# mir-group/allegro

Hardware: NVIDIA H100
Metric: atom-steps/sec (energy+forces) (higher is better)
Workload: dtype f32

## Files before the change

allegro_b200/_lib.py:

```python
from __future__ import annotations

import ctypes as C
import os
from typing import Optional, Sequence, Tuple

import torch

from . import build as _build

AB2_F64, AB2_F32, AB2_BF16 = 0, 1, 2
ACT_NONE, ACT_SILU, ACT_MUL_DSILU = 0, 1, 2
EPI_NONE, EPI_MUL_DSILU = 0, 1
NL_SILU, NL_MISH, NL_GELU = 1, 2, 3
NOT_ELIGIBLE = -1
MAX_SEG = 4

DTYPE_ENUM = {torch.float64: AB2_F64, torch.float32: AB2_F32, torch.bfloat16: AB2_BF16}
ACC_DTYPE = {torch.float64: torch.float64, torch.float32: torch.float32, torch.bfloat16: torch.float32}

_LIB: Optional[C.CDLL] = None

_vp, _i64, _i32, _dbl = C.c_void_p, C.c_int64, C.c_int, C.c_double

_SIGNATURES = {
# ... 2 lines not shown
    "ab2_last_error": ([], C.c_char_p),
    "ab2_set_option": ([C.c_char_p, _i32], C.c_int),
    "ab2_op_scatter_env": ([_i32, _i64, _i64, _dbl, _vp, _vp, _vp, _vp], C.c_int),
    "ab2_op_contract": ([_i32, _i32, _i64, _i32, _i32, _i32, _i32, _i32, _vp, _vp, _vp, _vp, _vp, _vp, _vp], C.c_int),
    "ab2_op_gather_rows": ([_i32, _i64, _i64, _dbl, _vp, _vp, _vp, _vp], C.c_int),
    "ab2_op_contract_wgrad": ([_i32, _i64, _i32, _i32, _i32, _i32, _i32, _vp, _vp, _vp, _vp, _vp, _vp, _vp], C.c_int),
    "ab2_sh_fwd": ([_i32, _i32, _i64, _vp, _vp, _vp], C.c_int),
    "ab2_sh_bwd": ([_i32, _i32, _i64, _vp, _vp, _vp, _i32, _vp], C.c_int),
    "ab2_linear": ([_i32, _i64, _i32, _i32, _i32, _vp, _vp, _vp, _vp, _vp, _i32, _vp, _vp, _i32, _vp, _vp, _vp, _vp, _i32, _vp, _i64, _vp], C.c_int),
    "ab2_linear_nl": ([_i32, _i64, _i32, _i32, _i32, _vp, _vp, _vp, _vp, _vp, _i32, _vp, _vp, _i32, _vp, _vp, _vp, _vp, _i32, _vp, _i64, _vp, _i32], C.c_int),
    "ab2_linear_packed_bytes": ([_i32, _i32, _i32], C.c_int64),
    "ab2_linear_pack": ([_i32, _i32, _i32, _vp, _vp, _vp], C.c_int),
    "ab2_mlp2_readout": ([_i32, _i32, _i64, _i32, _i32, _i32, _i32, _vp, _i64, _vp, _i64, _vp, _i64, _vp, _i64, _vp, _i64, _vp, _i64, _vp, _vp, _vp], C.c_int),
    "ab2_mlp2": ([_i32, _i32, _i64, _i32, _i32, _i32, _i32, _vp, _vp, _vp, _vp, _vp, _vp, _vp, _i64, _i32, _vp, _vp, _vp, _vp, _vp], C.c_int),
    "ab2_mlp2_nl": ([_i32, _i32, _i64, _i32, _i32, _i32, _i32, _vp, _vp, _vp, _vp, _vp, _vp, _vp, _i64, _i32, _vp, _vp, _vp, _vp, _vp, _i32], C.c_int),
    "ab2_mlp2_readout_nl": ([_i32, _i32, _i64, _i32, _i32, _i32, _i32, _vp, _i64, _vp, _i64, _vp, _i64, _vp, _i64, _vp, _i64, _vp, _i64, _vp, _vp, _vp, _i32],
                            C.c_int),
    "ab2_env_sum": ([_i32, _i32, _i64, _i32, _vp, _vp, _vp, _i64, _dbl, _vp, _vp], C.c_int),
    "ab2_env_bwd": ([_i32, _i32, _i64, _i64, _i32, _vp, _vp, _vp, _vp, _i64, _vp, _dbl, _vp, _i64, _vp, _vp], C.c_int),
    "ab2_tp_fwd": ([_i32, _i32, _i64, _i64, _i32, _i32, _i32, _i32, _vp, _vp, _vp, _vp, _vp, _vp, _i32, _vp, _vp, _i64, _vp, _vp], C.c_int),
    "ab2_tp_bwd": ([_i32, _i32, _i64, _i64, _i32, _i32, _i32, _i32, _vp, _vp, _vp, _vp, _vp, _vp, _i32, _vp, _vp, _i64, _vp, _vp, _vp, _i64, _vp, _vp, _vp], C.c_int),
    "ab2_tp_chain_fwd": ([_i32, _i32, _i64, _i64, _i32, _vp, _vp, _vp, _vp, _vp, _vp, _vp, _vp, _vp, _vp], C.c_int),
    "ab2_tp_chain_bwd": ([_i32, _i32, _i64, _i64, _i32, _vp, _vp, _vp, _vp, _vp, _vp, _vp, _vp, _vp, _vp, _vp, _vp, _vp, _vp], C.c_int),
    "ab2_edge_sum": ([_i32, _i64, _vp, _vp, _dbl, _vp, _vp], C.c_int),
    "ab2_edge_sum_bwd": ([_i32, _i64, _vp, _vp, _dbl, _vp, _vp], C.c_int),
    "ab2_force_scatter": ([_i32, _i64, _i64, _i64, _vp, _vp, _vp, _vp, _vp, _vp], C.c_int),
    "ab2_force_virial_scatter": ([_i32, _i64, _i64, _i64, _vp, _vp, _vp, _vp, _vp, _vp, _vp, _vp], C.c_int),
    "ab2_transpose_ui": ([_i32, _i64, _i32, _i32, _vp, _vp, _i32, _vp], C.c_int),
    "ab2_edge_vec": ([_i32, _i32, _i64, _vp, _vp, _vp, _vp, _vp, _vp], C.c_int),
    "ab2_radial_fwd": ([_i32, _i64, _i32, _i32, _dbl, _vp, _vp, _vp, _vp, _vp, _i32, _vp, _vp, _vp, _vp, _vp, _vp], C.c_int),
    "ab2_radial_pq_fwd": ([_i32, _i64, _i32, _i32, _dbl, _vp, _vp, _vp, _vp, _vp, _i32, _vp, _vp, _vp, _vp], C.c_int),
    "ab2_radial_pq_bwd": ([_i32, _i64, _i32, _i32, _dbl, _vp, _vp, _vp, _vp, _vp, _i32, _vp, _vp, _vp, _vp, _vp, _vp], C.c_int),
    "ab2_radial_pq_bwd_nl": ([_i32, _i64, _i32, _i32, _dbl, _vp, _vp, _vp, _vp, _vp, _i32, _vp, _vp, _vp, _vp, _vp, _vp, _i32], C.c_int),
    "ab2_zbl": ([_i32, _i64, _i32, _dbl, _dbl, _vp, _vp, _vp, _vp, _vp, _vp, _vp, _vp, _vp], C.c_int),
    "ab2_p2p_mailbox_bytes": ([_i32, _i32], C.c_int64),
    "ab2_p2p_alloc": ([_i64, C.POINTER(C.c_void_p)], C.c_int),
    "ab2_p2p_free": ([_vp], C.c_int),
    "ab2_p2p_get_handle": ([_vp, _vp], C.c_int),
    "ab2_p2p_open_handle": ([_vp, C.POINTER(C.c_void_p)], C.c_int),
    "ab2_p2p_close_handle": ([_vp], C.c_int),
    "ab2_p2p_error": ([_vp, _i32, _i32, _vp], C.c_int),
    "ab2_p2p_begin": ([_vp, _vp], C.c_int),
    "ab2_p2p_push_rows": ([_i32, _i32, _i32, _vp, _vp, _i32, _dbl, _vp, _i32, _i32, _vp, _vp, _vp], C.c_int),
    "ab2_p2p_push_rows_v": ([_i32, _i32, _i32, _vp, _vp, _i32, _dbl, _dbl, _dbl, _vp, _i32, _i32, _vp, _vp, _vp], C.c_int),
    "ab2_p2p_wait_unpack": ([_i32, _i32, _i32, _vp, _i32, _i32, _vp, _i32, _vp, _vp, _i32, _vp], C.c_int),
    "ab2_p2p_allreduce_energy": ([_vp, _i32, _i32, _i32, _vp, _vp, _vp, _vp, _vp], C.c_int),
    "ab2_p2p_mailbox_bytes_ex": ([_i32, _i32, _i32], C.c_int64),
    "ab2_p2p_push_rows_w": ([_i32, _i32, _vp, _vp, _i32, _vp, _i32, _i32, _vp, _vp, _vp], C.c_int),
    "ab2_p2p_wait_unpack_w": ([_i32, _i32, _vp, _i32, _i32, _vp, _i32, _vp, _vp, _vp, _vp], C.c_int),
    "ab2_p2p_allreduce_vec": ([_vp, _i32, _i32, _i32, _i32, _vp, _vp, _vp, _vp, _vp], C.c_int),
    "ab2_slab_plan_count": ([_i32, _i32, _i64, _vp, _vp, _vp, _i32, _i32, _dbl, _dbl, _dbl, _vp, _vp, _vp], C.c_int),
    "ab2_slab_plan_fill": ([_i64, _vp, _vp, _vp, _vp, _vp, _vp], C.c_int),
    "ab2_slab_plan_count_lattice": ([_i32, _i32, _i64, _vp, _vp, _vp, _i32, _i32, _dbl, _dbl, _vp, _vp, _vp], C.c_int),
    "ab2_nl_bin": ([_i32, _i64, _vp, _vp, _vp, _vp, _vp, _dbl, _vp, _vp], C.c_int),
    "ab2_nl_count": ([_i32, _i64, _vp, _vp, _vp, _vp, _vp, _dbl, _vp, _vp, _vp, _vp], C.c_int),
    "ab2_nl_fill": ([_i32, _i64, _vp, _vp, _vp, _vp, _vp, _dbl, _vp, _vp, _vp, _vp, _vp, _vp], C.c_int),
    "ab2_nl_lattice_bin": ([_i32, _i64, _vp, _vp, _vp, _vp, _vp, _vp, _dbl, _vp, _vp], C.c_int),
    "ab2_nl_lattice_count": ([_i32, _i64, _vp, _vp, _vp, _vp, _vp, _vp, _dbl, _vp, _vp, _vp, _vp], C.c_int),
    "ab2_nl_lattice_fill": ([_i32, _i64, _vp, _vp, _vp, _vp, _vp, _vp, _dbl, _vp, _vp, _vp, _vp, _vp, _vp], C.c_int),
    "ab2_radial_bwd": ([_i32, _i64, _i32, _i32, _dbl, _vp, _vp, _vp, _vp, _vp, _i32, _vp, _vp, _vp, _vp, _vp, _vp, _vp], C.c_int),
    "ab2_nl_frames_count": ([_i32, _i64, _i64, _vp, _vp, _vp, _vp, _vp, _vp, _dbl, _vp, _vp], C.c_int),
    "ab2_nl_frames_fill": ([_i32, _i64, _i64, _vp, _vp, _vp, _vp, _vp, _vp, _dbl, _vp, _vp, _vp, _vp], C.c_int),
    "ab2_nl_prune_count": ([_i32, _i64, _i64, _i32, _vp, _vp, _vp, _vp, _vp, _vp, _vp, _vp], C.c_int),
    "ab2_nl_prune_fill": ([_i32, _i64, _i64, _i32, _vp, _vp, _vp, _vp, _vp, _vp, _vp, _vp, _vp, _vp], C.c_int),
    "ab2_frame_scratch_elems": ([_i64, _i64], C.c_int64),
    "ab2_frame_sum": ([_i32, _i64, _i64, _vp, _vp, _vp, _i64, _vp, _vp], C.c_int),
# ... 686 lines not shown
    n_centres = n if n_centres is None else int(n_centres)
    dt = DTYPE_ENUM[pos.dtype]
    pos = _contig(pos, "pos")
    cell_id = torch.empty(n, dtype=torch.int32, device=pos.device)
    with _timed(name + "_bin"):
        _check(bin_fn(dt, n, _ptr(pos), *geom, _ptr(cell_id), _stream()))
    order = torch.argsort(cell_id, stable=True).to(torch.int32)
    ncells = ncell[0] * ncell[1] * ncell[2]
    cell_start = torch.zeros(ncells + 1, dtype=torch.int32, device=pos.device)
    cell_start[1:] = torch.cumsum(torch.bincount(cell_id.long(), minlength=ncells), 0).to(torch.int32)
    counts = torch.empty(n_centres, dtype=torch.int32, device=pos.device)
    with _timed(name + "_count"):
        _check(count_fn(dt, n_centres, _ptr(pos), *geom, _ptr(cell_start), _ptr(order), _ptr(counts), _stream()))
    row_ptr = torch.zeros(n_centres + 1, dtype=torch.int32, device=pos.device)
    row_ptr[1:] = torch.cumsum(counts, 0).to(torch.int32)
    E = int(row_ptr[-1])
    nbr = torch.empty(E, dtype=torch.int32, device=pos.device)
    shift = torch.empty(E, 3, dtype=pos.dtype, device=pos.device)
    if E:
        with _timed(name + "_fill"):
            _check(fill_fn(dt, n_centres, _ptr(pos), *geom, _ptr(cell_start), _ptr(order), _ptr(row_ptr), _ptr(nbr), _ptr(shift), _stream()))
    return row_ptr, nbr, shift


def radial_pq_fwd(dtype, S: int, p_cut: float, vec, ctr, nbr, types, rmax_table, bessel_w, PQ) -> torch.Tensor:
    E = ctr.shape[0]
    out = torch.empty(E, S, dtype=dtype, device=vec.device)
    with _timed("radial_fwd"):
        _check(load().ab2_radial_pq_fwd(DTYPE_ENUM[dtype], E, S, bessel_w.numel(), float(p_cut), _ptr(vec), _ptr(ctr), _ptr(nbr), _ptr(types),
                                        _ptr(rmax_table), rmax_table.shape[0], _ptr(bessel_w), _ptr(_contig(PQ, "PQ")), _ptr(out), _stream()))
    return out


def radial_pq_bwd(dtype, S: int, p_cut: float, vec, ctr, nbr, types, rmax_table, bessel_w, PQ, g_out, aux, gvec, nonlin: int = NL_SILU):
    E = ctr.shape[0]
    args = (DTYPE_ENUM[dtype], E, S, bessel_w.numel(), float(p_cut), _ptr(vec), _ptr(ctr), _ptr(nbr), _ptr(types), _ptr(rmax_table),
            rmax_table.shape[0], _ptr(bessel_w), _ptr(_contig(PQ, "PQ")), _ptr(_contig(g_out, "g_out")),
            _ptr(_contig(aux, "aux")) if aux is not None else None, _ptr(gvec), _stream())
    with _timed("radial_bwd"):
        _check(load().ab2_radial_pq_bwd(*args) if nonlin == NL_SILU else load().ab2_radial_pq_bwd_nl(*args, nonlin))


def _slab_plan(mode: int, pos: torch.Tensor, image: Optional[torch.Tensor], box, rank: int, world: int, width: float, jump: float,
               r_list: float, n_lists: int, rows=None):
    n = pos.shape[0]
    if rows is not None:
        rowsa = (C.c_double * 9)(*[float(v) for row in rows for v in row])
        count = lambda cls, counts: load().ab2_slab_plan_count_lattice(
            DTYPE_ENUM[pos.dtype], mode, n, _ptr(_contig(pos, "pos")) if n else None, _ptr(image) if n else None, rowsa, int(rank), int(world),
            float(jump), float(r_list), _ptr(cls), _ptr(counts), _stream())
        if n == 0:
            _check(count(None, None))
    else:
        boxa = (C.c_double * 3)(*[float(b) for b in box])
        count = lambda cls, counts: load().ab2_slab_plan_count(
            DTYPE_ENUM[pos.dtype], mode, n, _ptr(_contig(pos, "pos")), _ptr(image), boxa, int(rank), int(world), float(width), float(jump),
            float(r_list), _ptr(cls), _ptr(counts), _stream())
    if n == 0:
        return [torch.empty(0, dtype=torch.int64, device=pos.device) for _ in range(n_lists)], 0
    nblk = (n + 255) // 256
    cls = torch.empty(n, dtype=torch.uint8, device=pos.device)
    counts = torch.empty(nblk, 4, dtype=torch.int32, device=pos.device)
    with _timed("slab_plan_count"):
        _check(count(cls, counts))
    incl = torch.cumsum(counts, 0, dtype=torch.int32)
    offsets = (incl - counts).contiguous()
    lists = [torch.empty(n, dtype=torch.int64, device=pos.device) for _ in range(n_lists)]
    ptrs = [_ptr(t) for t in lists] + [None] * (3 - n_lists)
    with _timed("slab_plan_fill"):
        _check(load().ab2_slab_plan_fill(n, _ptr(cls), _ptr(offsets), *ptrs, _stream()))
    totals = incl[-1].tolist()
    return [t[:c] for t, c in zip(lists, totals)], int(totals[3])

# ... 343 lines not shown
```

allegro_b200/csrc/linear_tc.cu:

```cuda
#include <cuda.h>

#include <type_traits>

#include "common.cuh"

extern int g_ab2_opt_linear_tc;
extern int g_ab2_opt_linear_tma;
extern int g_ab2_opt_tc_debug;

namespace {

constexpr int BM = 128;
constexpr int KC = 32;
constexpr int NSTAGE = 4;
constexpr int RAW_STAGE = 256 * 4 * 16;
constexpr int EPI_LD = 40;
constexpr int NCONS = 8;
constexpr int EPI_BYTES = NCONS * 16 * EPI_LD * 4;
constexpr int STAGE_HALF = BM * KC * 2;
constexpr int NPROD = 8;
constexpr int NTHREADS = (NPROD + NCONS) * 32;
constexpr int MAX_W_BYTES = 128 * 1024;
constexpr int MAX_K = 512;
constexpr int MAX_N = 128;
constexpr int MAX_CHUNK = MAX_N / 32;
constexpr int TAIL_BARS = 2 * NSTAGE * 8, TAIL_CHUNK = MAX_CHUNK * 32, TAIL_KMAP = (MAX_K / 8) * 16;
constexpr int TAIL_BYTES = TAIL_BARS + TAIL_CHUNK + 2 * TAIL_KMAP;

struct TcSeg {
    const void* ptr;
    int64_t ld;
    int width;
    int accum;
    const void* aux;
    int64_t aux_ld;
};

// ... 815 lines not shown
    const int w_bytes = 2 * w_half;
    const int stage_bytes = 2 * STAGE_HALF;
    const int raw_slot = TMA_BOX_BYTES * (p.has_aux ? 2 : 1);
    uint8_t* sRaw = smem + ((1024u - (smem_u32(smem) & 1023u)) & 1023u);
    uint8_t* sW = sRaw + (size_t)NR * raw_slot;
    uint8_t* sA = sW + ((w_bytes + 127) & ~127);
    float* sEpi = reinterpret_cast<float*>(sA + p.nstage * stage_bytes);
    uint64_t* bars = reinterpret_cast<uint64_t*>(reinterpret_cast<uint8_t*>(sEpi) + EPI_BYTES);
    ChunkInfo* sChunk = reinterpret_cast<ChunkInfo*>(reinterpret_cast<uint8_t*>(bars) + TAIL_BARS);
    int4* sKseg = reinterpret_cast<int4*>(reinterpret_cast<uint8_t*>(sChunk) + TAIL_CHUNK);
    uint64_t* rbars = reinterpret_cast<uint64_t*>(reinterpret_cast<uint8_t*>(sKseg) + (MAX_K / 32) * 16);
    const uint32_t bar0 = smem_u32(bars), rbar0 = smem_u32(rbars);
    const int nkb = p.K / KC;

    if (threadIdx.x == 0) tma_init_bars(bar0, rbar0, WPG);
    if (threadIdx.x < MAX_K / 32) {
        sKseg[threadIdx.x] = tma_kseg_entry(p, threadIdx.x);
    } else if (threadIdx.x >= 64 && threadIdx.x < 64 + MAX_CHUNK) {
        sChunk[threadIdx.x - 64] = tc_chunk_info<TSrc>(p, (threadIdx.x - 64) * 32);
    }
    stage_w(sW, p.Wpacked, p.Wlo, w_half);
    fence_proxy_async();
    __syncthreads();
    TcCtx ctx;
    ctx.sW = sW; ctx.sA = sA; ctx.sEpi = sEpi; ctx.sChunk = sChunk; ctx.bar0 = bar0;
    ctx.nkb = nkb; ctx.stage_bytes = stage_bytes; ctx.w_half = w_half;
    const int64_t my_tiles = (p.num_tiles > blockIdx.x) ? (p.num_tiles - blockIdx.x + gridDim.x - 1) / gridDim.x : 0;
    const int64_t total = my_tiles * nkb;

    if (warp >= NPROD) {
        tc_consumer_role<TSrc, SPLIT, NCH, NL>(p, ctx, warp - NPROD, lane);
    } else {
        tma_converter_role<G, NL>(p, maps, NR, ctx, sRaw, sKseg, rbar0, total, warp, lane);
    }
}

constexpr int MLP2_MAX_H = 64;
constexpr int MLP2_CHUNK = 64;
constexpr int MLP2_MAX_CHUNKS = 4;
constexpr int MLP2_TAIL = TAIL_BARS + (1 + MLP2_MAX_CHUNKS) * TAIL_CHUNK + (MAX_K / 32) * 16 + 8 * 8;

struct Mlp2Params {
    TcParams s1;
    TcParams s2[MLP2_MAX_CHUNKS];
    int n0[MLP2_MAX_CHUNKS];
    int n2;
    int w2_npad;
    int backward;
    const float* pre;
    int64_t pre_ld;
    const float* gout1;
    int64_t gout1_ld;
    const float* w1row;
};

template <int NCH>
__device__ __forceinline__ void mlp2_stage2(const TcParams& p2, const ChunkInfo* chunks, float* stg, uint32_t h_u, uint32_t h_half, int H, uint32_t w_u,
                                            uint32_t w_half, int64_t tile, int wg, int w4, int lane) {
    float acc[16 * NCH];
    tc_mma_resident<NCH>(acc, h_u, h_half, H, w_u, w_half);
    tc_epilogue<float, NCH, false>(p2, chunks, stg, acc, tile, wg, w4, lane);
}

template <int NCH1, int NL>
__global__ void __launch_bounds__(NTHREADS, 1) mlp2_kernel(const __grid_constant__ Mlp2Params q, const __grid_constant__ TmaMaps maps, int NR) {
    constexpr int G = 2, WPG = NPROD / G;
// ... 741 lines not shown
        }
    }
    q.s2[0].Wpacked = W2_packed;
    q.s2[0].Wlo = reinterpret_cast<const uint8_t*>(W2_packed) + (size_t)w2_npad * H * 2;

    const unsigned grid = (unsigned)((num_tiles < num_sms) ? num_tiles : num_sms);
    cudaStream_t st = (cudaStream_t)stream;
    auto go = [&](auto kern) -> int {
        if (cudaFuncSetAttribute(kern, cudaFuncAttributeMaxDynamicSharedMemorySize, (int)smem) != cudaSuccess) {
            cudaGetLastError();
            return AB2_NOT_ELIGIBLE;
        }
        kern<<<grid, NTHREADS, smem, st>>>(q, maps, NR);
        AB2_CUDA_LAUNCH_CHECK();
        return 0;
    };
    return tc_with_nl(nonlin, [&](auto nl) -> int {
        constexpr int NL = decltype(nl)::value;
        switch (H / 32) {
            case 1: return go(mlp2_kernel<1, NL>);
            case 2: return go(mlp2_kernel<2, NL>);
        }
        return AB2_NOT_ELIGIBLE;
    });
}

extern "C" int ab2_mlp2(int dtype, int backward, int64_t M, int K, int H, int N, int n_a, const void* const* a_ptr, const int64_t* a_ld,
                        const int32_t* a_width, const void* W1_packed, const void* W2_packed, const void* w1_row, void* pre, int64_t pre_ld, int n_o,
                        void* const* o_ptr, const int64_t* o_ld, const int32_t* o_width, const int32_t* o_accum, void* stream) {
    return ab2_mlp2_nl(dtype, backward, M, K, H, N, n_a, a_ptr, a_ld, a_width, W1_packed, W2_packed, w1_row, pre, pre_ld, n_o, o_ptr, o_ld, o_width,
                       o_accum, stream, AB2_NL_SILU);
}

extern "C" int ab2_mlp2_readout_nl(int dtype, int backward, int64_t M, int P, int S, int U, int H, void* x, int64_t x_ld, void* s, int64_t s_ld,
                                   void* xl, int64_t xl_ld, void* pre_l, int64_t pre_l_ld, void* pre_r, int64_t pre_r_ld, void* ez, int64_t ez_ld,
                                   const void* const* w_packed, const void* w2_ro, void* stream, int nonlin) {
    AB2_CHECK_ARG(nonlin == AB2_NL_SILU || nonlin == AB2_NL_MISH || nonlin == AB2_NL_GELU, "nonlinearity");
    AB2_CHECK_ARG(P > 0 && S > 0 && U > 0 && H > 0 && M >= 0, "shape");
    AB2_CHECK_ARG(x && s && pre_l && pre_r && ez && w2_ro && w_packed && (backward || xl), "null pointer");
    AB2_CHECK_ARG(x_ld >= P && s_ld >= U && (backward || xl_ld >= S) && pre_l_ld >= H && pre_r_ld >= H && ez_ld >= 1, "leading dimension");
    if (M == 0) return 0;
    const int n_w = backward ? 3 : 4;
    auto al16 = [](const void* ptr, int64_t ld) { return (reinterpret_cast<uintptr_t>(ptr) % 16) == 0 && (ld * 4) % 16 == 0; };
    if (dtype != AB2_F32 || !g_ab2_opt_linear_tc || !g_ab2_opt_linear_tma || (!backward && !tc_encode_fn())) return AB2_NOT_ELIGIBLE;
    if (H != RO_H || S != RO_H || P % KC != 0 || U % KC != 0 || P + U > MAX_K || M >= ((int64_t)1 << 31)) return AB2_NOT_ELIGIBLE;
    if (!al16(x, x_ld) || !al16(s, s_ld) || (!backward && !al16(xl, xl_ld)) || !al16(pre_l, pre_l_ld) || !al16(pre_r, pre_r_ld) ||
        reinterpret_cast<uintptr_t>(w2_ro) % 16 != 0)
        return AB2_NOT_ELIGIBLE;
    for (int i = 0; i < n_w; ++i)
        if (!w_packed[i]) return AB2_NOT_ELIGIBLE;

    Mlp2RoParams q;
    memset(&q, 0, sizeof(q));
    const int64_t num_tiles = (M + BM - 1) / BM;
    q.P = P;
    q.w2ro = reinterpret_cast<const float*>(w2_ro);
    q.ez = reinterpret_cast<float*>(ez);
    q.ez_ld = ez_ld;
    for (int i = 0; i < n_w; ++i) q.w[i] = w_packed[i];
    TcParams& p = q.s1;
    p.M = M; p.num_tiles = num_tiles;
    auto out1 = [&](TcParams& o, void* ptr, int64_t ld, int n) {
        o.M = M; o.K = H; o.N = n; o.Npad = n; o.epi = AB2_EPI_NONE; o.num_tiles = num_tiles;
        o.n_o = 1; o.o[0].ptr = ptr; o.o[0].ld = ld; o.o[0].width = n;
    };
    int num_sms = 0, max_smem = 0;
// ... 68 lines not shown
```

allegro_b200/csrc/radial.cu:

```cuda
#include "common.cuh"

#define AB2_MAX_BESSEL 16

template <typename T>
__device__ __forceinline__ T ab2_sin(T x);
template <>
__device__ __forceinline__ float ab2_sin<float>(float x) { return sinf(x); }
template <>
__device__ __forceinline__ double ab2_sin<double>(double x) { return sin(x); }
template <typename T>
__device__ __forceinline__ T ab2_cos(T x);
template <>
__device__ __forceinline__ float ab2_cos<float>(float x) { return cosf(x); }
template <>
__device__ __forceinline__ double ab2_cos<double>(double x) { return cos(x); }
__device__ __forceinline__ float ab2_pow(float x, float p) { return powf(x, p); }
__device__ __forceinline__ double ab2_pow(double x, double p) { return pow(x, p); }

template <typename TPos, typename TAcc>
__global__ void __launch_bounds__(256) edge_vec_kernel(int64_t E, const TPos* __restrict__ pos, const int32_t* __restrict__ ctr,
                                                       const int32_t* __restrict__ nbr, const TPos* __restrict__ shift,
                                                       TAcc* __restrict__ vec) {
    const int64_t z = (int64_t)blockIdx.x * 256 + threadIdx.x;
    if (z >= E) return;
    const int64_t i = ctr[z], j = nbr[z];
#pragma unroll
    for (int a = 0; a < 3; ++a) {
        TPos d = pos[j * 3 + a] - pos[i * 3 + a];
        if (shift) d += shift[z * 3 + a];
        vec[z * 3 + a] = (TAcc)d;
    }
}

template <typename TAcc, bool GRAD>
__device__ __forceinline__ void bessel_basis(TAcc x, TAcc p, int nb, const TAcc* __restrict__ bw, TAcc* B, TAcc* dB) {
    const TAcc PI = TAcc(3.14159265358979323846);
    if (x >= TAcc(1)) {
        for (int n = 0; n < nb; ++n) {
            B[n] = TAcc(0);
            if (GRAD) dB[n] = TAcc(0);
        }
        return;
    }
    const TAcc xp = ab2_pow(x, p);
    const TAcc a = (p + 1) * (p + 2) / 2, b = p * (p + 2), c = p * (p + 1) / 2;
    const TAcc f = TAcc(1) - a * xp + b * xp * x - c * xp * x * x;
    const TAcc df = GRAD ? (-a * p * xp / x + b * (p + 1) * xp - c * (p + 2) * xp * x) : TAcc(0);
    const TAcc inv = TAcc(1) / (PI * x);
    for (int n = 0; n < nb; ++n) {
        const TAcc arg = PI * bw[n] * x;
        const TAcc s = ab2_sin(arg) * inv;
        B[n] = s * f;
        if (GRAD) {
            const TAcc ds = (bw[n] * ab2_cos(arg) - s) / x;
            dB[n] = ds * f + s * df;
        }
    }
}

template <typename TAct, typename TAcc>
__global__ void __launch_bounds__(256) radial_fwd_kernel(int64_t E, int S_rc, int nb, TAcc p, const TAcc* __restrict__ vec,
                                                         const int32_t* __restrict__ ctr, const int32_t* __restrict__ nbr,
                                                         const int32_t* __restrict__ types, const TAcc* __restrict__ rmax_table,
                                                         int num_types, const TAcc* __restrict__ bw, const TAcc* __restrict__ Wb,
                                                         const TAcc* __restrict__ cemb, const TAcc* __restrict__ nemb,
                                                         TAct* __restrict__ e0) {
    __shared__ TAcc sB[AB2_MAX_BESSEL][256];
    __shared__ int s_tc[256], s_tn[256];
    const int t = threadIdx.x;
    const int64_t z0 = (int64_t)blockIdx.x * 256;
    {
        const int64_t z = z0 + t;
        TAcc B[AB2_MAX_BESSEL];
        int tc = 0, tn = 0;
        if (z < E) {
            const TAcc vx = vec[z * 3], vy = vec[z * 3 + 1], vz = vec[z * 3 + 2];
            const TAcc r = sqrt(vx * vx + vy * vy + vz * vz);
            tc = types[ctr[z]];
            tn = types[nbr[z]];
            bessel_basis<TAcc, false>(r / rmax_table[tc * num_types + tn], p, nb, bw, B, nullptr);
        } else {
            for (int n = 0; n < nb; ++n) B[n] = TAcc(0);
        }
        for (int n = 0; n < nb; ++n) sB[n][t] = B[n];
        s_tc[t] = tc;
        s_tn[t] = tn;
    }
    __syncthreads();
    const int warp = t >> 5, lane = t & 31, half = S_rc >> 1;
// ... 437 lines not shown
```

allegro_b200/nn/_pipeline.py:

```python
from __future__ import annotations

import math
from typing import Dict, List, Optional

import torch

from .. import _lib
from ..data import EdgeCSR
from ._mlp import PackedMLP


def _env_perm(U: int, n_ir: int, individual: bool = True) -> torch.Tensor:
    r = torch.arange(n_ir).view(-1, 1)
    u = torch.arange(U).view(1, -1)
    if not individual:
        return (u + 0 * r).reshape(-1)
    return (u * n_ir + r).reshape(-1)


class _Saved:
    __slots__ = ("csr", "vec", "Y", "w0", "omega", "V", "gamma", "pre_lat", "pre_read", "X", "fold", "chain")


_BAKED_TABLES = {}
# ... 257 lines not shown
                ok = _lib.tp_chain_bwd(chain, l == 0, csr.row_ptr, csr.ctr, sv.gamma[0], sv.gamma[1] if l == 0 else None, sv.Y, sv.w0, g1,
                                       gV_last.view(E, U), gw0, gY if l == 0 else None, ggamma)
                if not ok:
                    raise RuntimeError("tp_chain_bwd declined a case its forward took")
                gV_in = None
            elif l == 0:
                gw0 = torch.empty(E, self.nw, dtype=dt, device=dev)
                _lib.tp_bwd(dt, self.lmax, N, E, U, ly["d_in"], ly["d_out"], ly["tab"], ly["cgw"], csr.row_ptr, csr.ctr,
                            sv.gamma[l], None, sv.Y, sv.w0, gV_next, None, gw0, gY, ggamma)
                gV_in = None
            else:
                gV_in = torch.empty(E, ly["d_in"], U, dtype=dt, device=dev)
                _lib.tp_bwd(dt, self.lmax, N, E, U, ly["d_in"], ly["d_out"], ly["tab"], ly["cgw"], csr.row_ptr, csr.ctr,
                            sv.gamma[l], sv.V[l], None, None, gV_next, gV_in, None, None, ggamma)
            gomega = torch.empty(E, self.nw, dtype=dt, device=dev)
            _lib.env_bwd(dt, self.lmax, U, csr.ctr, sv.Y, sv.omega[l], ggamma, self.sf, gomega, gY, row_ptr=csr.row_ptr)
            gV_next, gomega_next = gV_in, gomega
        _lib.set_tag("bwd.embed")
        gvec = _lib.sh_bwd(sv.vec, gY, self.lmax)
        if sv.fold:
            return gvec, [gw0, gX[:, :S], gomega_next]
        gx_emb = torch.empty(E, self.S_in, dtype=dt, device=dev)
        self.embed.backward([gw0, gX[:, :S], gomega_next], [], [gx_emb], [False])
        return gvec, gx_emb


class UpstreamPack:

    def __init__(self, edge_norm, radial, scalar_embed_mlp, dtype, device, fold_embed_of: Optional["AllegroCore"] = None):
        acc = _lib.ACC_DTYPE[dtype]
        self.fold = fold_embed_of is not None
        self.mlp = PackedMLP(scalar_embed_mlp, dtype, device, post=fold_embed_of.embed.W64[0] if self.fold else None)
        self.dtype = dtype
        self.S_rc = radial.out_dim
        self.kind = "spline" if hasattr(radial, "spline") else "bessel"
        if self.kind == "spline":
            sp = radial.spline
            self.num_types = radial.num_types
            self.rmax64 = edge_norm.rmax_table.detach().to(device=device, dtype=torch.float64).contiguous()
            self.sp_lower = sp.lower.detach().to(device=device, dtype=torch.float64)
            self.sp_upper = sp.upper.detach().to(device=device, dtype=torch.float64)
            self.sp_const = float(sp._const)
            self.sp_w = sp.flat_weights().to(device=device, dtype=torch.float64)
            return
        te = radial.type_embed
        self.p = float(radial.bessel_encode.p)
        self.S_rc = radial.out_dim
        self.rmax_table = edge_norm.rmax_table.detach().to(device=device, dtype=acc).contiguous()
        self.bessel_w = radial.bessel_encode.bessel_weights.detach().reshape(-1).to(device=device, dtype=acc).contiguous()
        self.Wb = te.basis_linear.folded_weights()[0].to(device=device, dtype=acc).contiguous()
        self.cemb = te.center_embed.weight.detach().to(device=device, dtype=acc).contiguous()
        self.nemb = te.neighbor_embed.weight.detach().to(device=device, dtype=acc).contiguous()
        self.PQ, self.S_pq, self.fold_radial = None, 0, False
        nb = int(self.bessel_w.numel())
        import os as _os

        if nb == 8 and _os.environ.get("ALLEGRO_B200_RADIAL_PQ", "1") == "1":
            Wb64 = te.basis_linear.folded_weights()[0].detach().double().cpu()
            ce, ne = te.center_embed.weight.detach().double().cpu(), te.neighbor_embed.weight.detach().double().cpu()
            T = ce.shape[0]
            temb = torch.cat([ce.unsqueeze(1).expand(T, T, -1), ne.unsqueeze(0).expand(T, T, -1)], dim=-1)
            PQ0 = temb.reshape(T * T, 1, -1) * Wb64.unsqueeze(0)
            if self.mlp.is_two_layer_nonlinear and self.mlp.dims[1] <= 128 and _os.environ.get("ALLEGRO_B200_FOLD_RADIAL", "1") == "1":
                self.fold_radial = True
                PQ0 = PQ0 @ self.mlp.W64[0]
            if PQ0.shape[-1] <= 128:
                self.PQ = PQ0.to(device=device, dtype=acc).contiguous()
                self.S_pq = int(PQ0.shape[-1])
            else:
                self.fold_radial = False

    def forward(self, vec, csr: EdgeCSR, types_i32, outs):
        dt = self.dtype
        if self.kind == "spline":
            from ._spline import spline_forward

            t64 = types_i32.long()
            e0, sp_saved = spline_forward(vec, t64[csr.ctr.long()], t64[csr.nbr.long()], self.rmax64, self.sp_lower, self.sp_upper, self.sp_const,
                                          self.sp_w, self.num_types, dt)
            return ("spline", sp_saved, self.mlp.forward([e0], outs))
        if self.fold_radial:
            h = _lib.radial_pq_fwd(dt, self.S_pq, self.p, vec, csr.ctr, csr.nbr, types_i32, self.rmax_table, self.bessel_w, self.PQ)
            _lib.linear([h], self.mlp.W[1], outs, act=_lib.ACT_SILU, W_packed=self.mlp.Wp[1], **self.mlp.nl_kw)
            return ("pq_fold", None, [h])
        if self.PQ is not None:
            e0 = _lib.radial_pq_fwd(dt, self.S_pq, self.p, vec, csr.ctr, csr.nbr, types_i32, self.rmax_table, self.bessel_w, self.PQ)
        else:
            e0 = _lib.radial_fwd(dt, self.S_rc, self.p, vec, csr.ctr, csr.nbr, types_i32, self.rmax_table, self.bessel_w, self.Wb, self.cemb, self.nemb)
        return ("bessel", None, self.mlp.forward([e0], outs))

    def backward(self, saved, gouts, vec, csr: EdgeCSR, types_i32, gvec):
        kind, sp_saved, pre = saved
        dt = self.dtype
        E = vec.shape[0]
        if kind == "pq_fold":
            g_h = self.mlp.hidden_grad(gouts)
            _lib.radial_pq_bwd(dt, self.S_pq, self.p, vec, csr.ctr, csr.nbr, types_i32, self.rmax_table, self.bessel_w, self.PQ, g_h, pre[0], gvec,
                               **self.mlp.nl_kw)
            return
        g_e0 = torch.empty(E, self.S_rc, dtype=dt, device=vec.device)
        if self.mlp.is_two_layer_nonlinear:
            self.mlp.backward_plain(gouts, pre, [g_e0])
        else:
            self.mlp.backward(gouts, pre, [g_e0], [False])
        if kind == "spline":
            from ._spline import spline_backward

            gvec += spline_backward(sp_saved, g_e0, self.sp_w, self.num_types).to(gvec.dtype)
        elif self.PQ is not None:
            _lib.radial_pq_bwd(dt, self.S_pq, self.p, vec, csr.ctr, csr.nbr, types_i32, self.rmax_table, self.bessel_w, self.PQ, g_e0, None, gvec)
        else:
            _lib.radial_bwd(dt, self.S_rc, self.p, vec, csr.ctr, csr.nbr, types_i32, self.rmax_table, self.bessel_w, self.Wb, self.cemb, self.nemb, g_e0, gvec)


def edge_energy_grad(core: "AllegroCore", up: UpstreamPack, csr: EdgeCSR, vec: torch.Tensor, types_i32: torch.Tensor,
                     gEi_scale: Optional[torch.Tensor], pair=None):
    dt = core.dtype
    E = csr.num_edges
    if up.fold:
        box = []
        Ei, X, Ez, sv = core.forward(csr, vec, None, fill_embed=lambda w0, x0, om0: box.append(up.forward(vec, csr, types_i32, [w0, x0, om0])))
        up_saved = box[0]
    else:
        x_emb = torch.empty(E, core.S_in, dtype=dt, device=vec.device)
        up_saved = up.forward(vec, csr, types_i32, [x_emb])
        Ei, X, Ez, sv = core.forward(csr, vec, x_emb)
    gEi = gEi_scale if gEi_scale is not None else torch.ones_like(Ei)
    gvec, gx_emb = core.backward(sv, gEi)
# ... 63 lines not shown
```

include/allegro_b200.h:

```cpp
#ifndef ALLEGRO_B200_H
#define ALLEGRO_B200_H
#include <stdint.h>

#ifdef __cplusplus
extern "C" {
#endif

enum { AB2_F64 = 0, AB2_F32 = 1, AB2_BF16 = 2 };
enum { AB2_ACT_NONE = 0, AB2_ACT_SILU = 1, AB2_ACT_MUL_DSILU = 2 };
enum { AB2_EPI_NONE = 0, AB2_EPI_MUL_DSILU = 1 };
enum { AB2_NL_SILU = 1, AB2_NL_MISH = 2, AB2_NL_GELU = 3 };

#define AB2_MAX_SEG 4
#define AB2_MAX_LMAX 4

const char* ab2_last_error(void);
int ab2_version(void);
int ab2_device_ok(void);
int ab2_set_option(const char* key, int value);


int ab2_op_scatter_env(int dtype, int64_t E, int64_t row , double sf,
                       const void* x2, const int64_t* idxs, void* gamma, void* stream);

// ... 182 lines not shown
                   const int64_t* Pe, const int32_t* row_ptr, const int32_t* nbr, int32_t* row_ptr_b, int32_t* cen_b,
                   int32_t* ctr_b, int32_t* nbr_b, void* vec_b, void* stream);
int ab2_fc3_fold(int acc_dtype, int64_t u0, int64_t U, double h, const int64_t* iptr, const int32_t* icen, const int32_t* ioff,
                 const int64_t* Pe, const int32_t* row_ptr, const int32_t* ctr, const int32_t* col_ptr, const int32_t* col_perm,
                 const int64_t* rptr, const int32_t* col, const void* gvec, double* blocks, void* stream);


#define AB2_FRAMES_MAX_ATOMS 4096

int ab2_slots_check(int pos_dtype, int64_t n, int64_t n_frames, const int32_t* frame_ptr, const void* pos, const void* pos_ref,
                    double half_skin, int32_t* frame_flag, void* stream);
int ab2_slots_count(int pos_dtype, int64_t n, int64_t n_frames, const int32_t* frame_ptr, const void* pos, const void* cell,
                    const void* inv_cell, const int32_t* pbc, const int32_t* nimg, double r_max, const int32_t* frame_flag,
                    int32_t* counts, void* stream);
int ab2_slots_place(int64_t n_frames, const int32_t* frame_ptr, const int32_t* slot_ptr, const int32_t* counts,
                    int32_t* frame_flag, int32_t* row_ptr, int32_t* overflow, int32_t* rebuilds, void* stream);
int ab2_slots_fill(int pos_dtype, int64_t n, int64_t n_frames, const int32_t* frame_ptr, const void* pos, const void* cell,
                   const void* inv_cell, const int32_t* pbc, const int32_t* nimg, double r_max, const int32_t* frame_flag,
                   const int32_t* row_ptr, double pad, int32_t* ctr, int32_t* nbr, void* shift, void* pos_ref, void* stream);
int ab2_slots_transpose(int64_t n_frames, int max_frame_atoms, const int32_t* frame_ptr, const int32_t* slot_ptr,
                        const int32_t* nbr, int32_t* frame_flag, int32_t* col_ptr, int32_t* col_perm, void* stream);

int ab2_radial_pq_fwd(int dtype, int64_t E, int S, int num_bessels, double p_cut, const void* vec,
                      const int32_t* ctr, const int32_t* nbr, const int32_t* types, const void* rmax_table,
                      int num_types, const void* bessel_w, const void* PQ, void* out, void* stream);
int ab2_radial_pq_bwd(int dtype, int64_t E, int S, int num_bessels, double p_cut, const void* vec,
                      const int32_t* ctr, const int32_t* nbr, const int32_t* types, const void* rmax_table,
                      int num_types, const void* bessel_w, const void* PQ, const void* g_out, const void* aux,
                      void* gvec, void* stream);
int ab2_radial_pq_bwd_nl(int dtype, int64_t E, int S, int num_bessels, double p_cut, const void* vec,
                         const int32_t* ctr, const int32_t* nbr, const int32_t* types, const void* rmax_table,
                         int num_types, const void* bessel_w, const void* PQ, const void* g_out, const void* aux,
                         void* gvec, void* stream, int nonlin);

int ab2_zbl(int acc_dtype, int64_t E, int num_types, double p_cut, double qq, const void* vec, const int32_t* ctr,
            const int32_t* nbr, const int32_t* types, const void* Z, const void* rmax_table, void* Ez, void* gvec,
            void* stream);

int ab2_sh_jvp(int acc_dtype, int lmax, int64_t E, const void* vec, const void* vdot, void* Yd, void* stream);
int ab2_sh_hvp(int acc_dtype, int lmax, int64_t E, const void* vec, const void* vdot, const void* gY, void* gvec_dot, void* stream);
int ab2_act_bwd_jvp(int dtype, int64_t n, const void* ga_dot, const void* ga, const void* pre, const void* pre_dot, void* out, int nonlin,
                    void* stream);
int ab2_radial_pq_jvp(int dtype, int64_t E, int S, int num_bessels, double p_cut, const void* vec, const void* vdot, const int32_t* ctr,
                      const int32_t* nbr, const int32_t* types, const void* rmax_table, int num_types, const void* bessel_w, const void* PQ,
                      void* out, void* stream);
int ab2_radial_jvp(int dtype, int64_t E, int S_rc, int num_bessels, double p_cut, const void* vec, const void* vdot, const int32_t* ctr,
                   const int32_t* nbr, const int32_t* types, const void* rmax_table, int num_types, const void* bessel_w, const void* Wb,
                   const void* center_embed, const void* neighbor_embed, void* e0_dot, void* stream);
int ab2_radial_pq_hvp(int dtype, int64_t E, int S, int num_bessels, double p_cut, const void* vec, const void* vdot, const int32_t* ctr,
                      const int32_t* nbr, const int32_t* types, const void* rmax_table, int num_types, const void* bessel_w, const void* PQ,
                      const void* g_out, const void* aux, void* gvec_dot, int nonlin, void* stream);
int ab2_radial_hvp(int dtype, int64_t E, int S_rc, int num_bessels, double p_cut, const void* vec, const void* vdot, const int32_t* ctr,
                   const int32_t* nbr, const int32_t* types, const void* rmax_table, int num_types, const void* bessel_w, const void* Wb,
                   const void* center_embed, const void* neighbor_embed, const void* g_e0, void* gvec_dot, void* stream);
int ab2_zbl_hvp(int acc_dtype, int64_t E, int num_types, double p_cut, double qq, const void* vec, const void* vdot, const int32_t* ctr,
                const int32_t* nbr, const int32_t* types, const void* Z, const void* rmax_table, void* gvec_dot, void* stream);
int ab2_fc_gather_tangent(int pos_dtype, int acc_dtype, int64_t u0, int64_t U, int64_t Cb, const void* pos, const void* shift,
                          const int64_t* atoms, const int64_t* cptr, const int32_t* cen, const int32_t* coff, const int64_t* ea,
                          const int32_t* row_ptr, const int32_t* nbr, const int64_t* Cp, const int64_t* Ep, int32_t* row_ptr_b,
                          int32_t* cen_b, int32_t* ctr_b, int32_t* nbr_b, void* vec_b, void* vdot_b, void* stream);
int ab2_fc_fold_tangent(int acc_dtype, int64_t u0, int64_t U, const int64_t* cptr, const int32_t* cen, const int32_t* coff,
                        const int64_t* ea, const int32_t* row_ptr, const int32_t* ctr, const int32_t* col_ptr, const int32_t* col_perm,
                        const int64_t* fptr, const int32_t* col, const int64_t* Ep, const void* gvec_dot, double* blocks, void* stream);


int64_t ab2_p2p_mailbox_bytes(int max_rows, int world);
// ... 43 lines not shown
```

Baseline: 3.511 million.

## Fuse radial hidden-grad GEMM with radial PQ backward in one TMA kernel

Adds a fused kernel that computes the MLP hidden-gradient GEMM on tensor cores and, in the consumer epilogue, recomputes the Bessel basis per edge and accumulates the radial adjoint straight into gvec. This drops the separate hidden_grad launch and the round trip of the E x S g_h intermediate through global memory. The PQ table is staged in shared memory, and the bessel helpers move into a shared header. The path only applies to f32 with 8 Bessels and S of 32 or 64, and falls back to the two-launch path otherwise. The epilogue adds per-edge transcendental and shuffle work to the GEMM consumers.

```diff
diff --git a/allegro_b200/_lib.py b/allegro_b200/_lib.py
--- a/allegro_b200/_lib.py
+++ b/allegro_b200/_lib.py
@@ -58,6 +58,8 @@
     "ab2_radial_pq_fwd": ([_i32, _i64, _i32, _i32, _dbl, _vp, _vp, _vp, _vp, _vp, _i32, _vp, _vp, _vp, _vp], C.c_int),
     "ab2_radial_pq_bwd": ([_i32, _i64, _i32, _i32, _dbl, _vp, _vp, _vp, _vp, _vp, _i32, _vp, _vp, _vp, _vp, _vp, _vp], C.c_int),
     "ab2_radial_pq_bwd_nl": ([_i32, _i64, _i32, _i32, _dbl, _vp, _vp, _vp, _vp, _vp, _i32, _vp, _vp, _vp, _vp, _vp, _vp, _i32], C.c_int),
+    "ab2_radial_pq_bwd_gemm": ([_i32, _i64, _i32, _i32, _i32, _vp, _vp, _vp, _vp, _i32, _dbl, _vp, _vp, _vp, _vp, _vp, _i32, _vp, _vp, _vp, _vp,
+                                _i32], C.c_int),
     "ab2_zbl": ([_i32, _i64, _i32, _dbl, _dbl, _vp, _vp, _vp, _vp, _vp, _vp, _vp, _vp, _vp], C.c_int),
     "ab2_p2p_mailbox_bytes": ([_i32, _i32], C.c_int64),
     "ab2_p2p_alloc": ([_i64, C.POINTER(C.c_void_p)], C.c_int),
@@ -810,13 +812,41 @@
     return out
 
 
-def radial_pq_bwd(dtype, S: int, p_cut: float, vec, ctr, nbr, types, rmax_table, bessel_w, PQ, g_out, aux, gvec, nonlin: int = NL_SILU):
+def radial_pq_bwd(dtype, S: int, p_cut: float, vec, ctr, nbr, types, rmax_table, bessel_w, PQ, g_out, aux, gvec, nonlin: int = NL_SILU,
+                  gemm: Optional[Tuple[Sequence[torch.Tensor], Optional[torch.Tensor]]] = None) -> bool:
     E = ctr.shape[0]
+    if gemm is not None:
+        gout_segs, W2T_packed = gemm
+        assert g_out is None and aux is not None and tuple(aux.shape) == (E, S)
+        if W2T_packed is None:
+            return False
+        na = len(gout_segs)
+        a_ptr = (C.c_void_p * na)()
+        a_ld = (C.c_int64 * na)()
+        a_w = (C.c_int32 * na)()
+        for s, t in enumerate(gout_segs):
+            t, ld = _row_strided(t, f"A segment {s}")
+            assert t.dtype == dtype and t.shape[0] == E
+            a_ptr[s], a_ld[s], a_w[s] = t.data_ptr(), ld, t.shape[1]
+            _ptr(t)
+        K = sum(int(w) for w in a_w)
+        timer = _timed("radial_pq_bwd_gemm")
+        args = (DTYPE_ENUM[dtype], E, K, S, na, a_ptr, a_ld, a_w, _ptr(W2T_packed), bessel_w.numel(), float(p_cut), _ptr(_contig(vec, "vec")),
+                _ptr(ctr), _ptr(nbr), _ptr(types), _ptr(rmax_table), rmax_table.shape[0], _ptr(bessel_w), _ptr(_contig(PQ, "PQ")),
+                _ptr(_contig(gvec, "gvec")), _stream(), int(nonlin))
+        with timer:
+            rc = load().ab2_radial_pq_bwd_gemm(*args)
+        if rc == NOT_ELIGIBLE:
+            timer.cancel()
+            return False
+        _check(rc)
+        return True
     args = (DTYPE_ENUM[dtype], E, S, bessel_w.numel(), float(p_cut), _ptr(vec), _ptr(ctr), _ptr(nbr), _ptr(types), _ptr(rmax_table),
             rmax_table.shape[0], _ptr(bessel_w), _ptr(_contig(PQ, "PQ")), _ptr(_contig(g_out, "g_out")),
             _ptr(_contig(aux, "aux")) if aux is not None else None, _ptr(gvec), _stream())
     with _timed("radial_bwd"):
         _check(load().ab2_radial_pq_bwd(*args) if nonlin == NL_SILU else load().ab2_radial_pq_bwd_nl(*args, nonlin))
+    return True
 
 
 def _slab_plan(mode: int, pos: torch.Tensor, image: Optional[torch.Tensor], box, rank: int, world: int, width: float, jump: float,
diff --git a/allegro_b200/csrc/linear_tc.cu b/allegro_b200/csrc/linear_tc.cu
--- a/allegro_b200/csrc/linear_tc.cu
+++ b/allegro_b200/csrc/linear_tc.cu
@@ -3,6 +3,7 @@
 #include <type_traits>
 
 #include "common.cuh"
+#include "radial_basis.cuh"
 
 extern int g_ab2_opt_linear_tc;
 extern int g_ab2_opt_linear_tma;
@@ -884,6 +885,144 @@
         tc_consumer_role<TSrc, SPLIT, NCH, NL>(p, ctx, warp - NPROD, lane);
     } else {
         tma_converter_role<G, NL>(p, maps, NR, ctx, sRaw, sKseg, rbar0, total, warp, lane);
+    }
+}
+
+constexpr int RADJ_NB = 8;
+
+struct RadialAdjParams {
+    const float* vec;
+    const int32_t* ctr;
+    const int32_t* nbr;
+    const int32_t* types;
+    const float* rmax_table;
+    const float* bw;
+    const float* PQ;
+    float* gvec;
+    int num_types;
+    float p;
+};
+
+template <int NCH, int NL>
+__device__ __forceinline__ void radial_adjoint_consumer_role(const TcParams& p, const TcCtx& c, const RadialAdjParams& ra, const float* sPQ, int cw,
+                                                             int lane) {
+    constexpr int H = 32 * NCH;
+    const int wg = cw >> 2, w4 = cw & 3;
+    const int r8 = lane >> 2, cq = 2 * (lane & 3);
+    int stage = 0;
+    uint32_t phase = 0;
+    float acc[16 * NCH];
+    auto row = [&](int64_t tile, int i) {
+        const int64_t m = tile * BM + wg * 64 + w4 * 16 + r8 + 8 * i;
+        return m < p.M ? m : p.M - 1;
+    };
+    int nc[2], nn[2];
+    auto fetch_idx = [&](int64_t tile) {
+        if (tile < p.num_tiles) {
+#pragma unroll
+            for (int i = 0; i < 2; ++i) {
+                nc[i] = __ldg(ra.ctr + row(tile, i));
+                nn[i] = __ldg(ra.nbr + row(tile, i));
+            }
+        }
+    };
+    fetch_idx(blockIdx.x);
+    for (int64_t tile = blockIdx.x; tile < p.num_tiles; tile += gridDim.x) {
+        int pair[2];
+        float v[2][3];
+#pragma unroll
+        for (int i = 0; i < 2; ++i) {
+            pair[i] = __ldg(ra.types + nc[i]) * ra.num_types + __ldg(ra.types + nn[i]);
+            const float* vr = ra.vec + row(tile, i) * 3;
+            v[i][0] = __ldg(vr); v[i][1] = __ldg(vr + 1); v[i][2] = __ldg(vr + 2);
+        }
+        fetch_idx(tile + gridDim.x);
+        tc_mma_ring<true, NCH>(acc, p, c, wg, lane, stage, phase);
+        float f[2];
+#pragma unroll
+        for (int i = 0; i < 2; ++i) {
+            const float r = sqrtf(v[i][0] * v[i][0] + v[i][1] * v[i][1] + v[i][2] * v[i][2]);
+            const float rmax = __ldg(ra.rmax_table + pair[i]);
+            float Bq[2], dBq[2];
+            bessel_basis<float, true>(r / rmax, ra.p, 2, ra.bw + cq, Bq, dBq);
+            float B[RADJ_NB], dB[RADJ_NB];
+#pragma unroll
+            for (int n = 0; n < RADJ_NB; ++n) {
+                B[n] = __shfl_sync(0xffffffffu, Bq[n & 1], (lane & ~3) | (n >> 1));
+                dB[n] = __shfl_sync(0xffffffffu, dBq[n & 1], (lane & ~3) | (n >> 1));
+            }
+            const float* m = sPQ + pair[i] * RADJ_NB * H + cq;
+            float gx = 0.f;
+#pragma unroll
+            for (int j = 0; j < 4 * NCH; ++j) {
+                float2 pq[RADJ_NB];
+#pragma unroll
+                for (int n = 0; n < RADJ_NB; ++n) pq[n] = *reinterpret_cast<const float2*>(m + n * H + 8 * j);
+                float h0 = 0.f, h1 = 0.f, s0 = 0.f, s1 = 0.f;
+#pragma unroll
+                for (int n = 0; n < RADJ_NB; ++n) {
+                    h0 = fmaf(B[n], pq[n].x, h0);
+                    h1 = fmaf(B[n], pq[n].y, h1);
+                    s0 = fmaf(dB[n], pq[n].x, s0);
+                    s1 = fmaf(dB[n], pq[n].y, s1);
+                }
+                gx = fmaf(acc[4 * j + 2 * i] * dact_f<NL>(h0), s0, gx);
+                gx = fmaf(acc[4 * j + 2 * i + 1] * dact_f<NL>(h1), s1, gx);
+            }
+            gx += __shfl_xor_sync(0xffffffffu, gx, 1);
+            gx += __shfl_xor_sync(0xffffffffu, gx, 2);
+            f[i] = gx / (rmax * r);
+        }
+        if ((lane & 3) == 0) {
+#pragma unroll
+            for (int i = 0; i < 2; ++i) {
+                const int64_t m = tile * BM + wg * 64 + w4 * 16 + r8 + 8 * i;
+                if (m < p.M) {
+                    float* g = ra.gvec + m * 3;
+                    g[0] += f[i] * v[i][0];
+                    g[1] += f[i] * v[i][1];
+                    g[2] += f[i] * v[i][2];
+                }
+            }
+        }
+    }
+}
+
+template <int G, int NCH, int NL>
+__global__ void __launch_bounds__(NTHREADS, 1) radial_adjoint_tma_kernel(const TcParams p, const __grid_constant__ TmaMaps maps, int NR,
+                                                                         const RadialAdjParams ra) {
+    constexpr int WPG = NPROD / G;
+    extern __shared__ __align__(1024) uint8_t smem[];
+    const int warp = __shfl_sync(0xffffffffu, threadIdx.x >> 5, 0), lane = threadIdx.x & 31;
+    const int w_half = p.Npad * p.K * 2;
+    const int w_bytes = 2 * w_half;
+    const int stage_bytes = 2 * STAGE_HALF;
+    uint8_t* sRaw = smem + ((1024u - (smem_u32(smem) & 1023u)) & 1023u);
+    uint8_t* sW = sRaw + (size_t)NR * TMA_BOX_BYTES;
+    uint8_t* sA = sW + ((w_bytes + 127) & ~127);
+    float* sPQ = reinterpret_cast<float*>(sA + p.nstage * stage_bytes);
+    uint64_t* bars = reinterpret_cast<uint64_t*>(reinterpret_cast<uint8_t*>(sPQ) + EPI_BYTES);
+    int4* sKseg = reinterpret_cast<int4*>(reinterpret_cast<uint8_t*>(bars) + TAIL_BARS + TAIL_CHUNK);
+    uint64_t* rbars = reinterpret_cast<uint64_t*>(reinterpret_cast<uint8_t*>(sKseg) + (MAX_K / 32) * 16);
+    const uint32_t bar0 = smem_u32(bars), rbar0 = smem_u32(rbars);
+    const int nkb = p.K / KC;
+
+    if (threadIdx.x == 0) tma_init_bars(bar0, rbar0, WPG);
+    if (threadIdx.x < MAX_K / 32) sKseg[threadIdx.x] = tma_kseg_entry(p, threadIdx.x);
+    const int n_pq = ra.num_types * ra.num_types * RADJ_NB * 32 * NCH;
+    for (int e = threadIdx.x; e < n_pq; e += NTHREADS) sPQ[e] = __ldg(ra.PQ + e);
+    stage_w(sW, p.Wpacked, p.Wlo, w_half);
+    fence_proxy_async();
+    __syncthreads();
+    TcCtx ctx;
+    ctx.sW = sW; ctx.sA = sA; ctx.sEpi = sPQ; ctx.sChunk = nullptr; ctx.bar0 = bar0;
+    ctx.nkb = nkb; ctx.stage_bytes = stage_bytes; ctx.w_half = w_half;
+    const int64_t my_tiles = (p.num_tiles > blockIdx.x) ? (p.num_tiles - blockIdx.x + gridDim.x - 1) / gridDim.x : 0;
+
+    if (warp >= NPROD) {
+        radial_adjoint_consumer_role<NCH, NL>(p, ctx, ra, sPQ, warp - NPROD, lane);
+    } else {
+        tma_converter_role<G, AB2_NL_SILU>(p, maps, NR, ctx, sRaw, sKseg, rbar0, my_tiles * nkb, warp, lane);
     }
 }
 
@@ -1691,6 +1830,76 @@
                        o_accum, stream, AB2_NL_SILU);
 }
 
+extern "C" int ab2_radial_pq_bwd_gemm(int dtype, int64_t M, int K, int H, int n_a, const void* const* a_ptr, const int64_t* a_ld,
+                                      const int32_t* a_width, const void* W_packed, int num_bessels, double p_cut, const void* vec,
+                                      const int32_t* ctr, const int32_t* nbr, const int32_t* types, const void* rmax_table, int num_types,
+                                      const void* bessel_w, const void* PQ, void* gvec, void* stream, int nonlin) {
+    AB2_CHECK_ARG(nonlin == AB2_NL_SILU || nonlin == AB2_NL_MISH || nonlin == AB2_NL_GELU, "nonlinearity");
+    AB2_CHECK_ARG(M >= 0, "shape");
+    if (M == 0) return 0;
+    AB2_CHECK_ARG(n_a >= 1 && n_a <= AB2_MAX_SEG, "segment count");
+    AB2_CHECK_ARG(K > 0 && H > 0 && num_types > 0, "shape");
+    int ks = 0;
+    for (int s = 0; s < n_a; ++s) {
+        AB2_CHECK_ARG(a_ptr[s] && a_width[s] > 0 && a_ld[s] >= a_width[s], "A segment");
+        ks += a_width[s];
+    }
+    AB2_CHECK_ARG(ks == K, "A segment widths must sum to K");
+    AB2_CHECK_ARG(vec && ctr && nbr && types && rmax_table && bessel_w && PQ && gvec, "null pointer");
+    auto al16 = [](const void* ptr, int64_t ld) { return (reinterpret_cast<uintptr_t>(ptr) % 16) == 0 && (ld * 4) % 16 == 0; };
+    if (dtype != AB2_F32 || !g_ab2_opt_linear_tc || !g_ab2_opt_linear_tma || !tc_encode_fn()) return AB2_NOT_ELIGIBLE;
+    if (num_bessels != RADJ_NB || (H != 32 && H != 64) || !W_packed || K % KC != 0 || K > MAX_K || M >= ((int64_t)1 << 31))
+        return AB2_NOT_ELIGIBLE;
+    if ((size_t)num_types * num_types * RADJ_NB * H * 4 > (size_t)EPI_BYTES) return AB2_NOT_ELIGIBLE;
+    for (int s = 0; s < n_a; ++s)
+        if (a_width[s] % KC != 0 || !al16(a_ptr[s], a_ld[s])) return AB2_NOT_ELIGIBLE;
+    int num_sms = 0, max_smem = 0;
+    tc_device_limits(num_sms, max_smem);
+    const int w_bytes = 2 * H * K * 2;
+    const int plans[2][2] = {{8, 4}, {4, 4}};
+    int NR = 0, nstage = 0;
+    size_t smem = 0;
+    for (int q = 0; q < 2 && !NR; ++q) {
+        const size_t need = 1024 + ((w_bytes + 127) & ~127) + (size_t)plans[q][1] * 2 * STAGE_HALF + EPI_BYTES + TAIL_BYTES +
+                            (size_t)plans[q][0] * TMA_BOX_BYTES;
+        if (need <= (size_t)max_smem) { NR = plans[q][0]; nstage = plans[q][1]; smem = need; }
+    }
+    if (!NR) return AB2_NOT_ELIGIBLE;
+
+    TcParams p;
+    memset(&p, 0, sizeof(p));
+    p.M = M; p.K = K; p.N = H; p.Npad = H; p.n_a = n_a; p.act = AB2_ACT_NONE; p.epi = AB2_EPI_NONE;
+    p.Wpacked = W_packed; p.Wlo = reinterpret_cast<const uint8_t*>(W_packed) + (size_t)H * K * 2;
+    p.num_tiles = (M + BM - 1) / BM; p.nstage = nstage; p.debug = g_ab2_opt_tc_debug;
+    TmaMaps maps;
+    memset(&maps, 0, sizeof(maps));
+    for (int s = 0; s < n_a; ++s) {
+        p.a[s].ptr = a_ptr[s]; p.a[s].ld = a_ld[s]; p.a[s].width = a_width[s];
+        if (!tc_make_map(&maps.a[s], a_ptr[s], a_ld[s], a_width[s], M)) return AB2_NOT_ELIGIBLE;
+    }
+    RadialAdjParams ra;
+    ra.vec = reinterpret_cast<const float*>(vec); ra.ctr = ctr; ra.nbr = nbr; ra.types = types;
+    ra.rmax_table = reinterpret_cast<const float*>(rmax_table); ra.bw = reinterpret_cast<const float*>(bessel_w);
+    ra.PQ = reinterpret_cast<const float*>(PQ); ra.gvec = reinterpret_cast<float*>(gvec);
+    ra.num_types = num_types; ra.p = (float)p_cut;
+
+    const unsigned grid = (unsigned)((p.num_tiles < num_sms) ? p.num_tiles : num_sms);
+    cudaStream_t st = (cudaStream_t)stream;
+    auto go = [&](auto kern) -> int {
+        if (cudaFuncSetAttribute(kern, cudaFuncAttributeMaxDynamicSharedMemorySize, (int)smem) != cudaSuccess) {
+            cudaGetLastError();
+            return AB2_NOT_ELIGIBLE;
+        }
+        kern<<<grid, NTHREADS, smem, st>>>(p, maps, NR, ra);
+        AB2_CUDA_LAUNCH_CHECK();
+        return 0;
+    };
+    return tc_with_nl(nonlin, [&](auto nl) -> int {
+        constexpr int NL = decltype(nl)::value;
+        return H == 32 ? go(radial_adjoint_tma_kernel<4, 1, NL>) : go(radial_adjoint_tma_kernel<4, 2, NL>);
+    });
+}
+
 extern "C" int ab2_mlp2_readout_nl(int dtype, int backward, int64_t M, int P, int S, int U, int H, void* x, int64_t x_ld, void* s, int64_t s_ld,
                                    void* xl, int64_t xl_ld, void* pre_l, int64_t pre_l_ld, void* pre_r, int64_t pre_r_ld, void* ez, int64_t ez_ld,
                                    const void* const* w_packed, const void* w2_ro, void* stream, int nonlin) {
diff --git a/allegro_b200/csrc/radial.cu b/allegro_b200/csrc/radial.cu
--- a/allegro_b200/csrc/radial.cu
+++ b/allegro_b200/csrc/radial.cu
@@ -1,21 +1,4 @@
-#include "common.cuh"
-
-#define AB2_MAX_BESSEL 16
-
-template <typename T>
-__device__ __forceinline__ T ab2_sin(T x);
-template <>
-__device__ __forceinline__ float ab2_sin<float>(float x) { return sinf(x); }
-template <>
-__device__ __forceinline__ double ab2_sin<double>(double x) { return sin(x); }
-template <typename T>
-__device__ __forceinline__ T ab2_cos(T x);
-template <>
-__device__ __forceinline__ float ab2_cos<float>(float x) { return cosf(x); }
-template <>
-__device__ __forceinline__ double ab2_cos<double>(double x) { return cos(x); }
-__device__ __forceinline__ float ab2_pow(float x, float p) { return powf(x, p); }
-__device__ __forceinline__ double ab2_pow(double x, double p) { return pow(x, p); }
+#include "radial_basis.cuh"
 
 template <typename TPos, typename TAcc>
 __global__ void __launch_bounds__(256) edge_vec_kernel(int64_t E, const TPos* __restrict__ pos, const int32_t* __restrict__ ctr,
@@ -29,32 +12,6 @@
         TPos d = pos[j * 3 + a] - pos[i * 3 + a];
         if (shift) d += shift[z * 3 + a];
         vec[z * 3 + a] = (TAcc)d;
-    }
-}
-
-template <typename TAcc, bool GRAD>
-__device__ __forceinline__ void bessel_basis(TAcc x, TAcc p, int nb, const TAcc* __restrict__ bw, TAcc* B, TAcc* dB) {
-    const TAcc PI = TAcc(3.14159265358979323846);
-    if (x >= TAcc(1)) {
-        for (int n = 0; n < nb; ++n) {
-            B[n] = TAcc(0);
-            if (GRAD) dB[n] = TAcc(0);
-        }
-        return;
-    }
-    const TAcc xp = ab2_pow(x, p);
-    const TAcc a = (p + 1) * (p + 2) / 2, b = p * (p + 2), c = p * (p + 1) / 2;
-    const TAcc f = TAcc(1) - a * xp + b * xp * x - c * xp * x * x;
-    const TAcc df = GRAD ? (-a * p * xp / x + b * (p + 1) * xp - c * (p + 2) * xp * x) : TAcc(0);
-    const TAcc inv = TAcc(1) / (PI * x);
-    for (int n = 0; n < nb; ++n) {
-        const TAcc arg = PI * bw[n] * x;
-        const TAcc s = ab2_sin(arg) * inv;
-        B[n] = s * f;
-        if (GRAD) {
-            const TAcc ds = (bw[n] * ab2_cos(arg) - s) / x;
-            dB[n] = ds * f + s * df;
-        }
     }
 }
 
diff --git a/allegro_b200/csrc/radial_basis.cuh b/allegro_b200/csrc/radial_basis.cuh
--- /dev/null
+++ b/allegro_b200/csrc/radial_basis.cuh
@@ -0,0 +1,46 @@
+#pragma once
+
+#include "common.cuh"
+
+#define AB2_MAX_BESSEL 16
+
+template <typename T>
+__device__ __forceinline__ T ab2_sin(T x);
+template <>
+__device__ __forceinline__ float ab2_sin<float>(float x) { return sinf(x); }
+template <>
+__device__ __forceinline__ double ab2_sin<double>(double x) { return sin(x); }
+template <typename T>
+__device__ __forceinline__ T ab2_cos(T x);
+template <>
+__device__ __forceinline__ float ab2_cos<float>(float x) { return cosf(x); }
+template <>
+__device__ __forceinline__ double ab2_cos<double>(double x) { return cos(x); }
+__device__ __forceinline__ float ab2_pow(float x, float p) { return powf(x, p); }
+__device__ __forceinline__ double ab2_pow(double x, double p) { return pow(x, p); }
+
+template <typename TAcc, bool GRAD>
+__device__ __forceinline__ void bessel_basis(TAcc x, TAcc p, int nb, const TAcc* __restrict__ bw, TAcc* B, TAcc* dB) {
+    const TAcc PI = TAcc(3.14159265358979323846);
+    if (x >= TAcc(1)) {
+        for (int n = 0; n < nb; ++n) {
+            B[n] = TAcc(0);
+            if (GRAD) dB[n] = TAcc(0);
+        }
+        return;
+    }
+    const TAcc xp = ab2_pow(x, p);
+    const TAcc a = (p + 1) * (p + 2) / 2, b = p * (p + 2), c = p * (p + 1) / 2;
+    const TAcc f = TAcc(1) - a * xp + b * xp * x - c * xp * x * x;
+    const TAcc df = GRAD ? (-a * p * xp / x + b * (p + 1) * xp - c * (p + 2) * xp * x) : TAcc(0);
+    const TAcc inv = TAcc(1) / (PI * x);
+    for (int n = 0; n < nb; ++n) {
+        const TAcc arg = PI * bw[n] * x;
+        const TAcc s = ab2_sin(arg) * inv;
+        B[n] = s * f;
+        if (GRAD) {
+            const TAcc ds = (bw[n] * ab2_cos(arg) - s) / x;
+            dB[n] = ds * f + s * df;
+        }
+    }
+}
diff --git a/allegro_b200/nn/_pipeline.py b/allegro_b200/nn/_pipeline.py
--- a/allegro_b200/nn/_pipeline.py
+++ b/allegro_b200/nn/_pipeline.py
@@ -313,6 +313,7 @@
         self.fold = fold_embed_of is not None
         self.mlp = PackedMLP(scalar_embed_mlp, dtype, device, post=fold_embed_of.embed.W64[0] if self.fold else None)
         self.dtype = dtype
+        self.bwd_path: Optional[str] = None
         self.S_rc = radial.out_dim
         self.kind = "spline" if hasattr(radial, "spline") else "bessel"
         if self.kind == "spline":
@@ -375,6 +376,12 @@
         dt = self.dtype
         E = vec.shape[0]
         if kind == "pq_fold":
+            if dt == torch.float32 and self.S_pq in (32, 64) and self.mlp.WTp[1] is not None and _lib.radial_pq_bwd(
+                    dt, self.S_pq, self.p, vec, csr.ctr, csr.nbr, types_i32, self.rmax_table, self.bessel_w, self.PQ, None, pre[0], gvec,
+                    gemm=(gouts, self.mlp.WTp[1]), **self.mlp.nl_kw):
+                self.bwd_path = "fused"
+                return
+            self.bwd_path = "two_launch"
             g_h = self.mlp.hidden_grad(gouts)
             _lib.radial_pq_bwd(dt, self.S_pq, self.p, vec, csr.ctr, csr.nbr, types_i32, self.rmax_table, self.bessel_w, self.PQ, g_h, pre[0], gvec,
                                **self.mlp.nl_kw)
diff --git a/include/allegro_b200.h b/include/allegro_b200.h
--- a/include/allegro_b200.h
+++ b/include/allegro_b200.h
@@ -238,6 +238,11 @@
                          const int32_t* ctr, const int32_t* nbr, const int32_t* types, const void* rmax_table,
                          int num_types, const void* bessel_w, const void* PQ, const void* g_out, const void* aux,
                          void* gvec, void* stream, int nonlin);
+int ab2_radial_pq_bwd_gemm(int dtype, int64_t M, int K, int H, int n_a, const void* const* a_ptr_host,
+                           const int64_t* a_ld_host, const int32_t* a_width_host, const void* W2T_packed, int num_bessels,
+                           double p_cut, const void* vec, const int32_t* ctr, const int32_t* nbr, const int32_t* types,
+                           const void* rmax_table, int num_types, const void* bessel_w, const void* PQ, void* gvec,
+                           void* stream, int nonlin);
 
 int ab2_zbl(int acc_dtype, int64_t E, int num_types, double p_cut, double qq, const void* vec, const int32_t* ctr,
             const int32_t* nbr, const int32_t* types, const void* Z, const void* rmax_table, void* Ez, void* gvec,
```

Result: faster. 3.646 million (median of 6 runs) (+3.8%).
